# blubs/OpenGLRaytracer

Hardware: AMD Instinct MI355X
Metric: primary Mrays/s at 1920×1080; achieved HBM GB/s vs peak; 1/2/4/8-GPU scaling (higher is better)
Workload: dtype f32

## Files before the change

openglraytracer_amd/csrc/rt_api.cpp:

```cpp
#include <hip/hip_runtime.h>

#include <algorithm>
#include <climits>
#include <cmath>
#include <cstdio>
#include <cstring>
#include <new>
#include <string>
#include <vector>

#include "build_id.h"
#include "rt_internal.h"

namespace rtamd {

namespace {
thread_local std::string g_error;
}

void set_error(const std::string &msg) { g_error = msg; }

int hip_fail(const char *what, hipError_t e) {
    set_error(std::string(what) + ": " + hipGetErrorString(e));
    return RT_ERR_HIP;
// ... 203 lines not shown
            e = hipMemcpyAsync(static_cast<float4 *>(nb) + base, olist.data(), olist.size(), hipMemcpyHostToDevice,
                               ctx->stream);
        if (e == hipSuccess) e = hipStreamSynchronize(ctx->stream);
        if (e == hipSuccess) e = await_scene_uses(scene, ctx->stream);
        if (e != hipSuccess) {
            (void)hipFreeAsync(nb, ctx->stream);
            return hip_fail("origin lists upload", e);
        }
        (void)hipFreeAsync(scene->dev.blob, ctx->stream);
        drop_scene_uses(scene);
        scene->dev.blob = nb;
        scene->capacity_units = static_cast<int32_t>(units);
    } else {
        e = hipMemcpyAsync(static_cast<float4 *>(scene->dev.blob) + base, olist.data(), olist.size(),
                           hipMemcpyHostToDevice, ctx->stream);
        if (e == hipSuccess) e = hipStreamSynchronize(ctx->stream);
        if (e != hipSuccess) return hip_fail("origin lists upload", e);
    }
    scene->dev.off_olist = static_cast<int32_t>(base);
    return RT_OK;
}

}

extern "C" {

const char *rt_last_error(void) { return g_error.c_str(); }

int rt_debug_scene_blob(const rt_object *objs, int n_objs, const rt_material *mats, int n_mats,
                        const rt_light *lights, int n_lights, void *out, long long cap, int32_t *meta) {
    std::vector<float4> blob;
    DeviceScene ds;
    const int rc = build_scene(objs, n_objs, mats, n_mats, lights, n_lights, blob, ds, true);
    if (rc != RT_OK) return rc;
    const long long bytes = static_cast<long long>(blob.size() * sizeof(float4));
    if (out && cap >= bytes) std::memcpy(out, blob.data(), static_cast<size_t>(bytes));
    if (meta) {
        const int32_t m[24] = {ds.blob_units, ds.off_spheres, ds.off_smeta, ds.off_boxes, ds.off_mats,
                               ds.off_lights, ds.off_lightmat, ds.off_bvh, ds.n_bvh, ds.off_blink, ds.off_cone,
                               ds.off_dmask, ds.dmask_n, ds.dmask_bytes, ds.off_gmask, ds.gmask_words,
                               ds.off_glist, ds.n_spheres, ds.n_boxes, ds.n_mats, ds.n_lights, ds.off_olist,
                               0, 0};
        std::memcpy(meta, m, sizeof m);
    }
    return static_cast<int>(bytes);
}
int rt_debug_launch_shape_n(const int32_t *f, int n) {
    if (!f || (n != 15 && n != 23)) return RT_ERR_INVALID;
    LaunchParams p{};
    int resident = 0;
    if (n == 23) {
        static const FrameView views[1] = {};
        static const float4 consts[1] = {};
        static int32_t sched[1] = {};
        p.n_views = f[15];
        p.views_dev = f[16] ? views : nullptr;
        p.consts_dev = f[16] ? consts : nullptr;
        p.sched = f[18] ? sched : nullptr;
        p.persistent0 = f[17] ? 0 : f[19];
        resident = f[20];
        p.shape_cull = f[21];
        p.off_dmask = f[22] > 0 ? 0 : -1;
        p.dmask_bytes = f[22];
        p.dmask_n = kShapeMaskTexels;
    }
    p.shape_launch = f[1];
    p.width = f[2];
    p.height = f[3];
    p.row_begin = f[4];
    p.n_rows = f[5];
    p.block_rows = f[6];
    p.n_shards = f[7];
    p.shard = f[8];
    p.out_format = f[9];
    p.n_frame_consts = f[10];
    p.cam_short = f[11];
    p.slice_begin = f[12];
    p.slice_rows = f[13];
    p.spp = f[14];
    return launch_shape(p, f[0], resident);
}
int rt_debug_launch_shape(const int32_t *f) { return rt_debug_launch_shape_n(f, 15); }
int rt_debug_last_queued(const rt_context *ctx) { return ctx ? (ctx->last_queued ? 1 : 0) : RT_ERR_INVALID; }
const char *rt_version(void) { return "openglraytracer_amd 0.3 (gfx950, " RT_BUILD_ID ")"; }

int rt_create(int device, rt_context **out) {
    if (!out) { set_error("rt_create: null out"); return RT_ERR_INVALID; }
    *out = nullptr;
    int n = 0;
    hipError_t e = hipGetDeviceCount(&n);
    if (e != hipSuccess || n <= 0) {
        set_error("rt_create: no HIP device");
        return RT_ERR_NO_DEVICE;
    }
    if (device < 0 || device >= n) {
        set_error("rt_create: device " + std::to_string(device) + " out of range");
        return RT_ERR_NO_DEVICE;
    }
    if ((e = hipSetDevice(device)) != hipSuccess) return hip_fail("hipSetDevice", e);
    rt_context *ctx = new (std::nothrow) rt_context;
    if (!ctx) { set_error("rt_create: out of memory"); return RT_ERR_NOMEM; }
    ctx->device = device;
    for (hipEvent_t &ev : ctx->sched_done)
        if ((e = hipEventCreateWithFlags(&ev, hipEventDisableTiming)) != hipSuccess) {
            rt_destroy(ctx);
            return hip_fail("rt_create", e);
        }
    if ((e = hipStreamCreateWithFlags(&ctx->stream, hipStreamDefault)) != hipSuccess ||
        (e = hipEventCreate(&ctx->ev0)) != hipSuccess || (e = hipEventCreate(&ctx->ev1)) != hipSuccess ||
        (e = hipDeviceGetAttribute(&ctx->n_cu, hipDeviceAttributeMultiprocessorCount, device)) != hipSuccess ||
        (e = hipMalloc(&ctx->sched, sizeof(int32_t) * kSchedInts * kSchedSlots)) != hipSuccess ||
        (e = hipMemset(ctx->sched, 0, sizeof(int32_t) * kSchedInts * kSchedSlots)) != hipSuccess ||
        (e = allow_large_lds(kMaxLds)) != hipSuccess) {
        rt_destroy(ctx);
        return hip_fail("rt_create", e);
    }
    int rc = check_kernarg_block(ctx->stream);
    if (rc != RT_OK) {
        rt_destroy(ctx);
        return rc;
    }
    *out = ctx;
    return RT_OK;
}

void rt_destroy(rt_context *ctx) {
    if (!ctx) return;
    (void)hipSetDevice(ctx->device);
    if (ctx->stream) (void)hipStreamSynchronize(ctx->stream);
    for (rt_scene *s : ctx->scenes) s->ctx = nullptr;
    for (hipEvent_t ev : ctx->sched_done)
        if (ev) (void)hipEventDestroy(ev);
    if (ctx->staging) (void)hipFree(ctx->staging);
    for (int s = 0; s < kBatchSlots; ++s) {
        if (ctx->batch_dev[s]) (void)hipFree(ctx->batch_dev[s]);
        if (ctx->batch_host[s]) (void)hipHostFree(ctx->batch_host[s]);
        if (ctx->batch_done[s]) (void)hipEventDestroy(ctx->batch_done[s]);
    }
    if (ctx->sched) (void)hipFree(ctx->sched);
    if (ctx->ev0) (void)hipEventDestroy(ctx->ev0);
    if (ctx->ev1) (void)hipEventDestroy(ctx->ev1);
    if (ctx->stream) (void)hipStreamDestroy(ctx->stream);
    delete ctx;
}

int rt_scene_create(rt_context *ctx, const rt_object *objs, int n_objs, const rt_material *mats, int n_mats,
                    const rt_light *lights, int n_lights, rt_scene **out) {
    if (!out) { set_error("rt_scene_create: null out"); return RT_ERR_INVALID; }
    *out = nullptr;
    if (!ctx || (n_objs > 0 && !objs) || n_objs < 0 || n_objs > RT_MAX_OBJECTS || !mats || n_mats <= 0 ||
        n_mats > RT_MAX_MATERIALS || n_lights < 0 || n_lights > RT_MAX_LIGHTS || (n_lights > 0 && !lights)) {
        set_error("rt_scene_create: bad arguments");
        return RT_ERR_INVALID;
    }
    std::vector<float4> blob;
    DeviceScene ds;
    int rc = build_scene(objs, n_objs, mats, n_mats, lights, n_lights, blob, ds);
    if (rc != RT_OK) return rc;
    LaunchParams probe{};
    probe.blob_units = ds.blob_units;
    probe.n_spheres = ds.n_spheres;
    probe.n_boxes = ds.n_boxes;
    const size_t lds = lds_bytes(probe);
    if (lds > kMaxLds) {
        set_error("rt_scene_create: scene needs " + std::to_string(lds) + " B of LDS (> 160 KiB)");
        return RT_ERR_UNSUPPORTED;
// ... 493 lines not shown
```

openglraytracer_amd/csrc/rt_internal.h:

```cpp
#pragma once

#include <hip/hip_runtime.h>

#include <cstdint>
#include <memory>
#include <string>
#include <vector>

#include "../../include/rt.h"

namespace rtamd {

struct SphereRec {
    float cx, cy, cz, rr;
};
struct SphereMeta {
    int32_t obj_index;
    int32_t material;
    float radius;
    int32_t pad;
};

struct BoxRec {
    float w2l[12];
// ... 45 lines not shown
constexpr int kOListSlots = 25;
constexpr int kOListRecordBytes = 32;
#ifndef RT_OLIST_FROM
#define RT_OLIST_FROM 33
#endif
constexpr int kOListMinSpheres = RT_OLIST_FROM;
constexpr float kOListBoundUnit = 1.0f / 256.0f;
struct BvhNode {
    float lo[3];
    int32_t skip;
    float hi[3];
    int32_t leaf;
};
static_assert(sizeof(BvhNode) == 32, "BvhNode layout");
constexpr int kBvhOctants = 8;

struct LightRec {
    float pos[3];
    float dead;
};

struct FrameView {
    float unproj[16];
    float proj[16];
    float origin[3];
    int32_t cull;
    const void *blob;
};
constexpr int kMaxViews = 8;
constexpr int kBatchSlots = 4;
constexpr int kMaxFrameConsts = 272;
constexpr int kMaxViewConsts = 256;
constexpr size_t kMaxLds = 160 * 1024;

struct LaunchParams {
    FrameView view[kMaxViews];
    int32_t n_views;
    int32_t width, height;
    int32_t row_begin, n_rows;
    int32_t block_rows, n_shards, shard;
    int32_t n_spheres, n_boxes, n_mats, n_lights;
    const void *scene;
    float4 *out;
    int32_t off_spheres, off_smeta, off_boxes, off_mats, off_lights, off_lightmat;
    int32_t off_bvh, n_bvh;
    int32_t off_blink;
    int32_t off_cone;
    int32_t off_dmask, dmask_n;
    int32_t dmask_bytes;
    int32_t off_gmask, gmask_words;
    int32_t off_glist;
    int32_t blob_units;
    int32_t spp, sample0, jitter;
    uint32_t seed;
    int32_t *sched;
    int32_t n_cu;
    int32_t out_format;
    int32_t n_frame_consts;
    int32_t cam_short;
    int32_t slice_begin, slice_rows;
    const FrameView *views_dev;
    const float4 *consts_dev;
    float4 frame_consts[kMaxFrameConsts];
    int32_t off_olist;
    int32_t dmask_box;
    int32_t off_bplane;
    int32_t shape_cull;
    int32_t scene_room;
    int32_t lean_views;
    int32_t shape_launch;
    int32_t persistent0;
};
static_assert(sizeof(LaunchParams) == 5808, "kernel argument block: the hidden arguments' offsets");
static_assert(sizeof(LaunchParams) <= 6144, "kernel argument block");
constexpr int kShapeMaskBytes = 15;
constexpr int kShapeMaskTexels = 12;
constexpr int kShapeRoom = 16;
constexpr int kShapeWide = 32;
int scene_shape(const LaunchParams &p, int max_depth);
constexpr int kLaunchPlain = 1;
constexpr int kLaunchPersistent = 2;
int launch_shape(const LaunchParams &p, int max_depth, int resident = 0);
#ifndef RT_CHUNK0
#define RT_CHUNK0 8
#endif
constexpr int kChunk0 = RT_CHUNK0;
#ifndef RT_TAIL_TILES0
#define RT_TAIL_TILES0 4
#endif
constexpr int kTailTiles0 = RT_TAIL_TILES0;
constexpr int kPersistentMinTilesPerWave = 192;
int persistent_groups(const LaunchParams &p, int resident);
constexpr bool kLeanViews(int shape) { return (shape & kShapeWide) != 0; }
inline int view_units(const LaunchParams &p) { return (p.lean_views ? 1 : 2) * p.n_spheres + p.n_boxes; }
constexpr int kQueues = 32;
constexpr int kQueueStride = 64;
constexpr int kSchedInts = 2 * kQueues * kQueueStride;
constexpr int kSchedSlots = 64;

struct DeviceScene {
    void *blob = nullptr;
    int32_t blob_units = 0;
    int32_t off_spheres = 0, off_smeta = 0, off_boxes = 0, off_mats = 0, off_lights = 0, off_lightmat = 0;
    int32_t off_bvh = 0, n_bvh = 0, off_blink = 0, off_cone = 0;
    int32_t off_dmask = -1, dmask_n = 0, dmask_bytes = 4;
    int32_t dmask_box = 0;
    int32_t off_bplane = -1;
    int32_t off_gmask = -1, gmask_words = 0, off_glist = -1;
    int32_t off_olist = -1;
    int32_t olist_eligible = 0;
    int32_t n_spheres = 0, n_boxes = 0, n_mats = 0, n_lights = 0;
    int32_t room = 0;
};

void host_frame_setup(LaunchParams &p, const float4 *const *blobs);
int host_view_consts(const LaunchParams &p, const FrameView &V, const float4 *blob, float4 *out);
bool fill_view(const rt_context *ctx, const rt_view &view, int width, int height, FrameView &out);

float gl_sin(float a);
float gl_cos(float a);
void reference_orbit(float time, float *speed, float pos[3], float *yaw);
void reference_view_gl(float time, float unproj[16], float view[16]);
void reference_box_transforms(const float pos[3], const float ang[3], float l2w[16], float w2l[16], float nrm[9]);

hipError_t launch_render(LaunchParams &p, int max_depth, hipStream_t stream);
size_t lds_bytes(const LaunchParams &p);
int queued_views(const LaunchParams &p, int max_depth);
int check_kernarg_block(hipStream_t stream);

void set_error(const std::string &msg);
int hip_fail(const char *what, hipError_t e);
struct UseEvent {
    hipEvent_t ev = nullptr;
    UseEvent() = default;
    UseEvent(const UseEvent &) = delete;
    UseEvent &operator=(const UseEvent &) = delete;
    ~UseEvent() {
        if (ev) (void)hipEventDestroy(ev);
    }
};
int check_render_args(const rt_context *ctx, const rt_scene *scene, int width, int height, int max_depth);
LaunchParams base_params(const rt_context *ctx, const rt_scene *scene, const rt_view *views, int n_views,
                         int width, int height);
int launch(rt_context *ctx, LaunchParams &p, int max_depth, hipStream_t stream);
int ensure_origin_lists(rt_context *ctx, const rt_scene *scene, int max_depth);
int note_scene_use(const rt_scene *scene, hipStream_t stream, std::shared_ptr<UseEvent> *shared = nullptr);
inline size_t surface_bytes(int fmt) { return fmt == RT_OUTPUT_RGBA8 ? 4 : (fmt == RT_OUTPUT_RGB32F ? 12 : 16); }

}

struct rt_context {
    int device = 0;
    hipStream_t stream = nullptr;
    hipEvent_t ev0 = nullptr, ev1 = nullptr;
    float4 *staging = nullptr;
    size_t staging_px = 0;
    bool timed = false;
    int culling = 1;
    int timing = 1;
    int output = RT_OUTPUT_RGBA32F;
    int host_consts = 1;
    int origin_lists = 1;
    int scene_shapes = 1;
    int launch_shapes = 1;
    int persistent0 = 1;
    void *batch_dev[rtamd::kBatchSlots] = {};
    void *batch_host[rtamd::kBatchSlots] = {};
    hipEvent_t batch_done[rtamd::kBatchSlots] = {};
    bool batch_used[rtamd::kBatchSlots] = {};
    unsigned batch_next = 0;
    int n_cu = 0;
    int32_t *sched = nullptr;
    unsigned sched_next = 0;
    hipEvent_t sched_done[rtamd::kSchedSlots] = {};
    bool sched_used[rtamd::kSchedSlots] = {};
    bool last_queued = false;
    std::vector<struct rt_scene *> scenes;
};

struct rt_scene {
    int device = 0;
// ... 15 lines not shown
```

openglraytracer_amd/csrc/rt_kernel.hip:

```cpp
#include <hip/hip_runtime.h>

#include <algorithm>
#include <climits>
#include <cstdint>
#include <string>

#include "rt_internal.h"

namespace rtamd {
namespace {

constexpr int kWavesX = 2, kWavesY = 2;
constexpr int kTileX = 8 * kWavesX, kTileY = 8 * kWavesY;
constexpr int kThreads = 64 * kWavesX * kWavesY;

struct v3 {
    float x, y, z;
};
__device__ __forceinline__ v3 mk(float x, float y, float z) { return {x, y, z}; }
__device__ __forceinline__ v3 add(v3 a, v3 b) { return {a.x + b.x, a.y + b.y, a.z + b.z}; }
__device__ __forceinline__ v3 sub(v3 a, v3 b) { return {a.x - b.x, a.y - b.y, a.z - b.z}; }
__device__ __forceinline__ v3 muls(v3 a, float s) { return {a.x * s, a.y * s, a.z * s}; }
__device__ __forceinline__ v3 sel(bool c, v3 a, v3 b) { return {c ? a.x : b.x, c ? a.y : b.y, c ? a.z : b.z}; }
__device__ __forceinline__ float dot(v3 a, v3 b) { return a.x * b.x + (a.y * b.y + a.z * b.z); }
// ... 828 lines not shown
            const int s = base + __builtin_ctzll(mask);
            mask &= mask - 1;
            exact(s);
            if (!wave_any(need && !hit)) return hit;
        }
    }
    return hit;
}

__device__ __forceinline__ bool occluded(const Scene &S, v3 start, v3 dir, v3 p, v3 L, int light, int slot,
                                         uint64_t mask, bool need, const uint4 *pre = nullptr) {
    RT_CYC(kCycShadow);
    const bool hit = occluded_impl(S, start, dir, p, L, light, slot, mask, need, pre);
    RT_CYC_AFTER(kCycPhong, hit ? 1 : 0);
    return hit;
}

struct Collision {
    v3 p, n;
    bool inside;
    int material;
};

template <bool kPrimary>
__device__ __forceinline__ Collision resolve_impl(const Scene &S, const Ray &r, const Hit &h, bool valid) {
    Collision c;
    c.p = mk(0.0f, 0.0f, 0.0f);
    c.n = mk(0.0f, 0.0f, 1.0f);
    c.inside = false;
    c.material = 0;
    if (!valid) return c;
    if (h.slot >= 0) {
        const float4 sp = S.sph[h.slot];
        const v3 pos = mk(sp.x, sp.y, sp.z);
        c.material = S.smeta[h.slot].y;
        c.p = add(r.start, muls(r.dir, h.t));
        c.n = normalize(sub(c.p, pos));
        c.inside = h.info & 1;
        if (c.inside) c.n = muls(c.n, -1.0f);
    } else {
        const BoxRec &B = S.box[~h.slot];
        c.material = B.material;
        v3 rs;
        if (kPrimary) {
            const float4 bc = S.box_cam[~h.slot];
            rs = mk(bc.x, bc.y, bc.z);
        } else {
            rs = xform_point(B.w2l, r.start);
        }
        const v3 rd = box_dir(B, r.dir);
        c.inside = h.info & 1;
        const int face = h.info >> 1;
        v3 n = mk(face == 0 ? 1.0f : 0.0f, face == 1 ? 1.0f : 0.0f, face == 2 ? 1.0f : 0.0f);
        if (comp(rd, face) > 0.0f) n = muls(n, -1.0f);
        const float *N = B.nrm;
        c.n = mk(N[0] * n.x + N[1] * n.y + N[2] * n.z, N[3] * n.x + N[4] * n.y + N[5] * n.z,
                 N[6] * n.x + N[7] * n.y + N[8] * n.z);
        const v3 lp = add(rs, muls(rd, h.t));
        c.p = xform_point(B.l2w, lp);
    }
    return c;
}
template <bool kPrimary>
__device__ __forceinline__ Collision resolve(const Scene &S, const Ray &r, const Hit &h, bool valid) {
    RT_CYC(kCycResolve);
    const Collision c = resolve_impl<kPrimary>(S, r, h, valid);
    RT_CYC_AFTER(kCycWalk, c.p.x);
    return c;
}

#ifdef RT_PHASE_TRACE
constexpr unsigned kPhaseWaves = 1u << 17;
__device__ unsigned long long rt_phase_buf[kPhaseWaves * 16];
#define RT_PHASE(k)                                                                                        \
    do {                                                                                                    \
        const unsigned long long now_ = __builtin_amdgcn_s_memrealtime();                                   \
        const unsigned wg_ = (blockIdx.y * gridDim.x + blockIdx.x) * (kThreads / 64) + (threadIdx.x >> 6); \
        if ((threadIdx.x & 63) == 0 && wg_ < kPhaseWaves) rt_phase_buf[wg_ * 16 + (k)] = now_;              \
    } while (0)
#define RT_PHASE_AFTER(k, v)                     \
    do {                                         \
        if ((v) != -12345) RT_PHASE(k);      \
    } while (0)
#else
#define RT_PHASE_AFTER(k, v) \
    do {                     \
    } while (0)
#define RT_PHASE(k) \
    do {            \
    } while (0)
#endif

template <bool kUni = false>
__device__ __forceinline__ v3 phong_impl(const Scene &S, const Ray &r, const Collision &c, bool valid, int umat = 0) {
#if defined(RT_UNIFORM_MAT) && !defined(RT_UNIFORM_MAT_LM_ONLY)
    const MatRec m = kUni ? cload(S.cmat + umat) : S.mat[c.material];
#else
    const MatRec &m = S.mat[c.material];
#endif
    float4 dif = make_float4(0.0f, 0.0f, 0.0f, 0.0f), spe = dif;
    const v3 view = normalize_unit(muls(r.dir, -1.0f));
    int slot = -1;
    for (int j = 0; j < S.nl; ++j) {
        const LightRec L = cload(S.clight + j);
        if (L.dead != 0.0f) continue;
        ++slot;
        const v3 lpos = mk(L.pos[0], L.pos[1], L.pos[2]);
        const v3 sdir = sub(lpos, c.p);
        int ptexel = -1;
        uint4 pre = make_uint4(0u, 0u, 0u, 0u);
        if (S.glist) {
            ptexel = valid ? direction_texel(kGMaskTexels, muls(sdir, -1.0f)) : -1;
            if (ptexel >= 0) pre = S.glist[static_cast<size_t>(slot) * 6 * kGMaskTexels * kGMaskTexels + ptexel];
        }
        const v3 ldir = normalize(sdir);
        const float cos_theta = dot(ldir, c.n);
        const v3 nl = muls(ldir, -1.0f);
        const v3 lref = normalize_unit(sub(nl, muls(c.n, 2.0f * -cos_theta)));
        const float cos_phi = dot(view, lref);
#ifdef RT_UNIFORM_MAT
        const LightMatRec q = kUni ? cload(S.clm + (umat * S.nl + j)) : S.lm[c.material * S.nl + j];
#else
        const LightMatRec &q = S.lm[c.material * S.nl + j];
#endif
        const float kd = gmax(cos_theta, 0.0f);
        const float xs = gmax(cos_phi, 0.0f);
        const bool need_pow = !((xs == 0.0f) & (m.shininess > 0.0f));
        float ks = 0.0f;
        if (wave_any(need_pow && valid)) ks = need_pow ? glsl_pow_cos(xs, m.shininess) : 0.0f;
        const float4 nd = make_float4(dif.x + q.ld_md[0] * kd, dif.y + q.ld_md[1] * kd, dif.z + q.ld_md[2] * kd,
                                      dif.w + q.ld_md[3] * kd);
        const float4 ns = make_float4(spe.x + q.ls_ms[0] * ks, spe.y + q.ls_ms[1] * ks, spe.z + q.ls_ms[2] * ks,
                                      spe.w + q.ls_ms[3] * ks);
        const bool changes = (q.always != 0) | ((kd != 0.0f) & (q.d_nz != 0)) | ((ks != 0.0f) & (q.s_nz != 0));
        const bool need = valid && changes;
        if (j == 1) RT_PHASE(5);
#ifdef RT_ABLATE_SHADOW
        if (need) { dif = nd; spe = ns; }
        continue;
#endif
        if (wave_any(need)) {
            uint64_t smask = 0u;
            if (S.glist)
                smask = static_cast<uint64_t>(static_cast<int64_t>(ptexel));
            else if (S.gmask && need)
                smask = static_cast<uint64_t>(static_cast<int64_t>(direction_texel(kGMaskTexels, muls(sdir, -1.0f))));
            else if (S.dmask && !S.gmask)
                smask = direction_mask(S.dmask + slot * 6 * S.dmask_n * S.dmask_n * S.dmask_bytes, S.dmask_n,
                                       S.dmask_bytes, muls(sdir, -1.0f), S.ns + (S.dmask_box ? S.nb : 0));
            const bool shadowed = occluded(S, add(c.p, muls(c.n, 0.01f)), sdir, c.p, lpos, j, slot, smask, need,
                                           S.glist ? &pre : nullptr);
            if (need && !shadowed) {
                dif = nd;
                spe = ns;
            }
        }
    }
    RT_PHASE(6);
    const float px = ((m.amb_sum[0] + dif.x) + spe.x) + m.emissive[0];
    const float py = ((m.amb_sum[1] + dif.y) + spe.y) + m.emissive[1];
    const float pz = ((m.amb_sum[2] + dif.z) + spe.z) + m.emissive[2];
    const float pw = ((m.amb_sum[3] + dif.w) + spe.w) + m.emissive[3];
    return mk(px * pw, py * pw, pz * pw);
}
__device__ __forceinline__ v3 phong(const Scene &S, const Ray &r, const Collision &c, bool valid) {
    RT_CYC(kCycPhong);
    const v3 col = phong_impl(S, r, c, valid);
    RT_CYC_AFTER(kCycWalk, col.x);
    return col;
}

__device__ __forceinline__ v3 trace0(const Scene &S, const Ray &r, bool valid) {
// ... 353 lines not shown
        __builtin_assume(S.gmask != nullptr);
        __builtin_assume(S.glist != nullptr);
        __builtin_assume(S.olist != nullptr);
    }
    if constexpr ((kShape & kShapeRoom) != 0) {
        S.nb = 1;
        S.room = 1;
        S.dmask_box = 0;
        S.cbplane = nullptr;
    }
    RT_CYC(kCycRaygen);
    if (!wave_any(px.active)) return;
    const int x = px.x, y = px.y, local_row = px.local_row;
    const bool active = px.active;
    constexpr bool kPlain = (kLaunch & kLaunchPlain) != 0;
    static_assert(!kPlain || (kDepth == 0 && !kAccum && (kShape & kShapeMaskBytes) != 0),
                  "plain launches: the depth-0 shaped kernels, no accumulation");
    const int lr0 = (kPlain ? 0 : p.slice_begin) + wy * 8;
    S.tx0 = wx * 8;
    S.tx1 = S.tx0 + 7;
    if (kPlain || p.n_shards <= 0 || (p.block_rows % 8 == 0 && lr0 % 8 == 0)) {
        S.ty0 = output_row<kLaunch>(p, lr0);
        S.ty1 = S.ty0 + 7;
    } else {
        S.ty0 = INT_MAX;
        S.ty1 = INT_MIN;
        for (int i = 0; i < 8; ++i) {
            const int fy = output_row(p, lr0 + i);
            S.ty0 = fy < S.ty0 ? fy : S.ty0;
            S.ty1 = fy > S.ty1 ? fy : S.ty1;
        }
    }
    float4 *out = p.out + static_cast<size_t>(z) * p.n_rows * p.width;
    const uint32_t idx = static_cast<uint32_t>(local_row) * static_cast<uint32_t>(p.width) + static_cast<uint32_t>(x);

    if constexpr (!kAccum) {
        const Ray ray = have_pre ? pre : camera_ray<kLaunch>(p, V, x, y, 0.0f, 0.0f);
#if defined(RT_ABLATE_RAYGEN)
        (void)ray;
        const v3 col = mk(float(x), float(y), 0.0f);
#elif defined(RT_ABLATE_TRACE)
        const v3 col = ray.dir;
#else
        if constexpr (kDepth > 0) {
            trace_tree<kDepth>(S, ray, active, [&](v3 col) { store_pixel(p, z, idx, col); });
            return;
        }
        const v3 col = trace0(S, ray, active);
#endif
        RT_CYC_AFTER(kCycStore, col.x);
        if (active) store_pixel<kLaunch>(p, z, idx, col);
    } else {
        const uint32_t pixel = static_cast<uint32_t>(y) * static_cast<uint32_t>(p.width) + static_cast<uint32_t>(x);
        v3 acc = mk(0.0f, 0.0f, 0.0f);
        for (int smp = 0; smp < p.spp; ++smp) {
            const uint32_t sid = static_cast<uint32_t>(p.sample0 + smp);
            const float jx = p.jitter ? jitter_u(p.seed, sid, pixel, 0u) : 0.0f;
            const float jy = p.jitter ? jitter_u(p.seed, sid, pixel, 1u) : 0.0f;
            v3 col = mk(0.0f, 0.0f, 0.0f);
            if constexpr (kDepth == 0) col = trace0(S, camera_ray(p, V, x, y, jx, jy), active);
            else trace_tree<kDepth>(S, camera_ray(p, V, x, y, jx, jy), active, [&](v3 c) { col = c; });
            acc = add(acc, col);
        }
        if (active) {
            const float4 o = out[idx];
            out[idx] = make_float4(o.x + acc.x, o.y + acc.y, o.z + acc.z, o.w + 0.0f);
        }
    }
}

constexpr bool kQueuedDepth(int depth) { return depth >= 2; }

using LaunchArgs = const __attribute__((address_space(4))) LaunchParams *;
__device__ __forceinline__ const LaunchParams &launch_args() {
    LaunchArgs a = (LaunchArgs)__builtin_amdgcn_kernarg_segment_ptr();
    asm volatile("" : "+s"(a));
    return *(const LaunchParams *)a;
}
__device__ __forceinline__ float4 *persistent_slot(const LaunchParams &p, float4 *lds) {
    return lds + p.blob_units + __builtin_amdgcn_readfirstlane(threadIdx.x >> 6) * p.n_frame_consts;
}
__device__ __forceinline__ void persistent_refill(const LaunchParams &p, float4 *lds, int z) {
    float4 *const slot = persistent_slot(p, lds);
    __builtin_amdgcn_fence(__ATOMIC_RELEASE, "wavefront");
    __builtin_amdgcn_wave_barrier();
    int lane = threadIdx.x & 63;
    asm volatile("" : "+v"(lane));
    for (int i = lane; i < p.n_frame_consts; i += 64) slot[i] = p.consts_dev[z * p.n_frame_consts + i];
    __builtin_amdgcn_fence(__ATOMIC_ACQUIRE, "wavefront");
    __builtin_amdgcn_wave_barrier();
}
template <int kShape, int kLaunch>
__device__ __forceinline__ void persistent_tile(const LaunchParams &p, float4 *lds, int z, int wx, int wy) {
    const float4 *blob = static_cast<const float4 *>(p.scene);
    float4 *const slot = persistent_slot(p, lds);
    Scene S;
    S.sph = lds + p.off_spheres;
    S.smeta = reinterpret_cast<const int4 *>(lds + p.off_smeta);
    S.sph_cam = slot;
    S.sph_px = reinterpret_cast<const int4 *>(slot + p.n_spheres);
    S.box = reinterpret_cast<const BoxRec *>(lds + p.off_boxes);
    S.box_cam = slot + 2 * p.n_spheres;
    S.mat = reinterpret_cast<const MatRec *>(lds + p.off_mats);
    S.light = reinterpret_cast<const LightRec *>(lds + p.off_lights);
    S.lm = reinterpret_cast<const LightMatRec *>(lds + p.off_lightmat);
    S.bvh = lds + p.off_bvh;
    S.blink = reinterpret_cast<const uint32_t *>(lds + p.off_blink);
    S.cone = nullptr;
    S.dmask = reinterpret_cast<const char *>(lds + p.off_dmask);
    S.dmask_n = kShapeMaskTexels;
    S.dmask_bytes = kShape & kShapeMaskBytes;
    S.dmask_box = p.dmask_box;
    S.cbplane = p.off_bplane >= 0 ? (const __attribute__((address_space(4))) float4 *)(blob + p.off_bplane) : nullptr;
    S.gmask = nullptr;
    S.gwords = 0;
    S.glist = nullptr;
    S.olist = nullptr;
    S.cbox = (const __attribute__((address_space(4))) BoxRec *)(blob + p.off_boxes);
    S.clight = (const __attribute__((address_space(4))) LightRec *)(blob + p.off_lights);
#ifdef RT_UNIFORM_MAT
    S.cmat = (const __attribute__((address_space(4))) MatRec *)(blob + p.off_mats);
    S.clm = (const __attribute__((address_space(4))) LightMatRec *)(blob + p.off_lightmat);
#endif
    S.nbvh = 0;
    S.ns = p.n_spheres;
    S.nb = p.n_boxes;
    S.nl = p.n_lights;
    S.nm = p.n_mats;
    const FrameView V = cload((const __attribute__((address_space(4))) FrameView *)(p.views_dev) + z);
    const Ray none{mk(0.0f, 0.0f, 0.0f), mk(0.0f, 0.0f, 0.0f)};
    render_wave_tile<0, false, kShape, kLaunch>(p, S, V, wx, wy, z, wave_pixel<kLaunch>(p, wx, wy), none, false);
}
template <int kShape, int kLaunch>
__device__ __forceinline__ void render_persistent0(float4 *lds) {
    static_assert((kLaunch & kLaunchPlain) != 0 && (kShape & kShapeMaskBytes) != 0, "plain shaped launches");
    __builtin_amdgcn_s_setprio(1);
    {
        const LaunchParams &p = launch_args();
        const float4 *blob = static_cast<const float4 *>(p.scene);
        for (int i = threadIdx.x; i < p.blob_units; i += kThreads) lds[i] = blob[i];
    }
    __syncthreads();
    __builtin_amdgcn_s_setprio(0);
    const auto global_wave = [] {
        return static_cast<int>(blockIdx.x) * (kThreads / 64) + __builtin_amdgcn_readfirstlane(threadIdx.x >> 6);
    };
    const auto queue_waves = [](int q) {
        return (static_cast<int>(gridDim.x) * (kThreads / 64) - q + kQueues - 1) / kQueues;
    };
    int held = -1;
    int c = global_wave();
    for (;;) {
        int t, t_end, z, wx, wy;
        {
            const LaunchParams &p = launch_args();
            const int wtx = (p.width + 7) / 8, view_tiles = wtx * ((p.height + 7) / 8);
            const int total = view_tiles * p.n_views;
            const int tail_max = kTailTiles0 * static_cast<int>(gridDim.x) * (kThreads / 64);
            const int body = (total - (total < tail_max ? total : tail_max)) / kChunk0;
            if (c >= body + (total - body * kChunk0)) break;
            const int q = global_wave() % kQueues;
            int nxt = 0;
            if ((threadIdx.x & 63) == 0) nxt = atomicAdd(p.sched + q * kQueueStride, 1);
            t = c < body ? c * kChunk0 : body * kChunk0 + (c - body);
            t_end = c < body ? t + kChunk0 : t + 1;
            z = t / view_tiles;
            const int r = t - z * view_tiles;
            wy = r / wtx;
            wx = r - wy * wtx;
            if (z != held) persistent_refill(p, lds, z);
            held = z;
            c = (queue_waves(q) + __builtin_amdgcn_readfirstlane(nxt)) * kQueues + q;
        }
        for (; t < t_end; ++t) {
            const LaunchParams &p = launch_args();
            if (z != held) persistent_refill(p, lds, z);
            held = z;
            persistent_tile<kShape, kLaunch>(p, lds, z, wx, wy);
            if (++wx == (p.width + 7) / 8) {
                wx = 0;
                if (++wy == (p.height + 7) / 8) {
                    wy = 0;
                    ++z;
                }
            }
        }
    }
    const LaunchParams &p = launch_args();
    const int q = global_wave() % kQueues;
    if ((threadIdx.x & 63) == 0 && atomicAdd(p.sched + (kQueues + q) * kQueueStride, 1) == queue_waves(q) - 1) {
        atomicExch(p.sched + q * kQueueStride, 0);
        atomicExch(p.sched + (kQueues + q) * kQueueStride, 0);
    }
}

template <int kDepth, bool kAccum, bool kDev = false, int kShape = 0, int kLaunch = 0>
__global__ __launch_bounds__(kThreads) RT_OCCUPANCY void render_kernel(LaunchParams p) {
    constexpr bool kPlain = (kLaunch & kLaunchPlain) != 0;
    extern __shared__ __attribute__((aligned(16))) float4 lds[];
    if constexpr ((kLaunch & kLaunchPersistent) != 0) {
        static_assert(kPlain && kDev && kDepth == 0 && !kAccum, "persistent: plain depth-0 device-view batches");
        render_persistent0<kShape, kLaunch>(lds);
        return;
    }
    __builtin_amdgcn_s_setprio(1);
    const bool queued = kQueuedDepth(kDepth) && !kDev && p.sched != nullptr;
    const int z = queued ? 0 : static_cast<int>(blockIdx.z);
    const int n_staged = queued ? p.n_views : 1;
    FrameView Vdev;
    if constexpr (kDev) Vdev = cload((const __attribute__((address_space(4))) FrameView *)(p.views_dev) + z);
    const FrameView &V = kDev ? Vdev : p.view[z];
    const int wave = __builtin_amdgcn_readfirstlane(threadIdx.x >> 6), lane = threadIdx.x & 63;
    RT_PHASE(0);
#ifdef RT_PHASE_TRACE
    {
        const unsigned wg_ = (blockIdx.y * gridDim.x + blockIdx.x) * (kThreads / 64) + (threadIdx.x >> 6);
        const unsigned hw = __builtin_amdgcn_s_getreg((31 << 11) | 4), xcc = __builtin_amdgcn_s_getreg((31 << 11) | 20);
        if ((threadIdx.x & 63) == 0 && wg_ < kPhaseWaves) {
            rt_phase_buf[wg_ * 16 + 8] = hw;
            rt_phase_buf[wg_ * 16 + 9] = xcc;
        }
    }
#endif
    const float4 *blob = static_cast<const float4 *>(V.blob ? V.blob : p.scene);
    const int tid = threadIdx.x;
    float4 first = make_float4(0.0f, 0.0f, 0.0f, 0.0f), fc = first;
    if (tid < p.blob_units) first = blob[tid];
    static_assert(kMaxViewConsts <= kThreads, "one record per thread");
    constexpr bool kLean = kLeanViews(kShape);
    const int skip = kLean ? p.n_spheres : 0, keep = p.n_frame_consts - skip;
    if (tid < keep) fc = (kDev ? p.consts_dev : p.frame_consts)[z * p.n_frame_consts + skip + tid];
    float4 *const views = lds + p.blob_units;
    float4 *sph_cam = kLean ? nullptr : views;
    int4 *sph_px = reinterpret_cast<int4 *>(views + (kLean ? 0 : p.n_spheres));
    float4 *box_cam = reinterpret_cast<float4 *>(sph_px + p.n_spheres);
    const int own_wx = static_cast<int>(blockIdx.x) * kWavesX + wave % kWavesX;
    const int own_wy = static_cast<int>(blockIdx.y) * kWavesY + wave / kWavesX;
    const Pixel own = wave_pixel<kLaunch>(p, own_wx, own_wy);
    RT_PHASE_AFTER(14, own.y);
    Ray own_ray{mk(0.0f, 0.0f, 0.0f), mk(0.0f, 0.0f, 0.0f)};
    if (!queued && !kAccum) own_ray = camera_ray<kLaunch>(p, V, own.x, own.y, 0.0f, 0.0f);
    RT_PHASE_AFTER(15, own_ray.dir.x + own_ray.dir.y + own_ray.dir.z);
    RT_PHASE(10);
    if (tid < p.blob_units) lds[tid] = first;
    RT_PHASE(11);
    for (int i = tid + kThreads; i < p.blob_units; i += kThreads) lds[i] = blob[i];
    const int view_units = (kLean ? 1 : 2) * p.n_spheres + p.n_boxes;
    if (kPlain || p.n_frame_consts > 0) {
        if (tid < keep) views[tid] = fc;
        if (kLean) {
            for (int i = tid + keep; i < n_staged * keep; i += kThreads) {
                const int k = i / keep;
                views[i] = p.frame_consts[k * p.n_frame_consts + skip + (i - k * keep)];
            }
        } else {
            for (int i = tid + p.n_frame_consts; i < n_staged * p.n_frame_consts; i += kThreads)
                views[i] = p.frame_consts[i];
        }
    } else {
        frame_setup(p, V, sph_cam, sph_px, box_cam);
        for (int k = 1; k < n_staged; ++k) {
            float4 *c = views + k * view_units;
            int4 *px = reinterpret_cast<int4 *>(c + (kLean ? 0 : p.n_spheres));
            frame_setup(p, p.view[k], kLean ? nullptr : c, px, reinterpret_cast<float4 *>(px + p.n_spheres));
        }
    }
    RT_PHASE(12);
#ifdef RT_STATS
    if (lane < kStats) rt_stats_lds[wave][lane] = 0u;
#endif
#ifdef RT_CYCLES
    if (lane <= kCycPhases) rt_cyc_lds[wave][lane] = lane == kCycPhases ? __builtin_amdgcn_s_memtime() : 0u;
// ... 151 lines not shown
}

template <bool kAccum, bool kDev, int kShape>
hipError_t launch_shaped0(LaunchParams &p, hipStream_t stream) {
    if constexpr (!kAccum) {
        if ((launch_shape(p, 0) & kLaunchPlain) != 0) {
            if constexpr (kDev) {
                constexpr int kPersistent = kLaunchPlain | kLaunchPersistent;
                const size_t lds = persistent_lds_bytes(p);
                if (p.persistent0 > 0 && p.sched && lds <= kMaxLds && p.n_cu > 0) {
                    const void *fn = reinterpret_cast<const void *>(&render_kernel<0, false, true, kShape, kPersistent>);
                    const int groups = persistent_groups(p, groups_per_cu(fn, lds) * p.n_cu);
                    if (groups > 0) {
                        p.lean_views = 0;
                        hipLaunchKernelGGL((render_kernel<0, false, true, kShape, kPersistent>), dim3(groups),
                                           dim3(kThreads), lds, stream, p);
                        return hipGetLastError();
                    }
                }
            }
            return launch_kernel<0, false, kDev, kShape, kLaunchPlain>(p, stream);
        }
    }
    return launch_kernel<0, kAccum, kDev, kShape>(p, stream);
}
template <bool kAccum, bool kDev>
hipError_t launch_depth0(LaunchParams &p, hipStream_t stream) {
    switch (scene_shape(p, 0)) {
        case 2: return launch_shaped0<kAccum, kDev, 2>(p, stream);
        case 4: return launch_shaped0<kAccum, kDev, 4>(p, stream);
        case 8: return launch_shaped0<kAccum, kDev, 8>(p, stream);
        case 2 | kShapeRoom: return launch_shaped0<kAccum, kDev, 2 | kShapeRoom>(p, stream);
        case 4 | kShapeRoom: return launch_shaped0<kAccum, kDev, 4 | kShapeRoom>(p, stream);
        case 8 | kShapeRoom: return launch_shaped0<kAccum, kDev, 8 | kShapeRoom>(p, stream);
        default: return launch_kernel<0, kAccum, kDev, 0>(p, stream);
    }
}

template <int kDepth>
hipError_t launch_deep(LaunchParams &p, hipStream_t stream) {
    switch (scene_shape(p, kDepth)) {
        case kShapeWide: return launch_kernel<kDepth, false, false, kShapeWide>(p, stream);
        case kShapeWide | kShapeRoom: return launch_kernel<kDepth, false, false, kShapeWide | kShapeRoom>(p, stream);
        default: return launch_kernel<kDepth, false, false, 0>(p, stream);
    }
}

template <int kDepth>
hipError_t launch_depth(LaunchParams &p, hipStream_t stream) {
    if (p.views_dev) {
        if constexpr (kDepth == 0) {
            if (p.spp == 0) return launch_depth0<false, true>(p, stream);
        } else if constexpr (kDepth == 1) {
            if (p.spp == 0) return launch_kernel<kDepth, false, true>(p, stream);
        }
        return hipErrorInvalidValue;
    }
    if constexpr (kDepth == 0) return p.spp > 0 ? launch_depth0<true, false>(p, stream) : launch_depth0<false, false>(p, stream);
    if constexpr (kDepth >= 2) {
        if (p.spp == 0) return launch_deep<kDepth>(p, stream);
    }
    return p.spp > 0 ? launch_kernel<kDepth, true>(p, stream) : launch_kernel<kDepth, false>(p, stream);
}

}

int scene_shape(const LaunchParams &p, int max_depth) {
    if (!p.shape_cull) return 0;
    const int box = p.n_boxes == 1 && p.scene_room ? kShapeRoom : 0;
    if (max_depth == 0) {
        if (p.off_dmask < 0 || (p.dmask_bytes != 2 && p.dmask_bytes != 4 && p.dmask_bytes != 8) ||
            p.dmask_n != kShapeMaskTexels)
            return 0;
        return p.dmask_bytes | box;
    }
    if (max_depth >= 2) {
        if (p.off_gmask < 0 || p.off_glist < 0 || p.off_olist < 0) return 0;
        return kShapeWide | box;
    }
    return 0;
}

int persistent_groups(const LaunchParams &p, int resident) {
#if defined(RT_STATS) || defined(RT_CYCLES) || defined(RT_PHASE_TRACE)
    return 0;
#endif
    if (p.persistent0 <= 0 || (launch_shape(p, 0) & kLaunchPlain) == 0 || scene_shape(p, 0) == 0) return 0;
    if (!p.views_dev || !p.consts_dev || p.n_views <= kMaxViews || !p.sched) return 0;
    const bool forced = p.persistent0 >= 8;
    const int groups = forced && p.persistent0 < resident ? p.persistent0 : resident;
    const long long waves = static_cast<long long>(groups) * (kThreads / 64);
    const long long tiles = static_cast<long long>((p.width + 7) / 8) * ((p.height + 7) / 8) * p.n_views;
    if (waves < kQueues || tiles >= (1ll << 30)) return 0;
    if (!forced && tiles < kPersistentMinTilesPerWave * waves) return 0;
    return groups;
}

int launch_shape(const LaunchParams &p, int max_depth, int resident) {
    if (resident > 0) {
        const int shape = launch_shape(p, max_depth);
        return shape | (shape != 0 && persistent_groups(p, resident) > 0 ? kLaunchPersistent : 0);
    }
    if (!p.shape_launch || max_depth != 0 || p.spp > 0) return 0;
    const int slice_rows = p.slice_rows > 0 ? p.slice_rows : p.n_rows;
    const int slice_begin = p.slice_rows > 0 ? p.slice_begin : 0;
    const bool plain = p.n_shards <= 0 && p.row_begin == 0 && p.n_rows == p.height && slice_begin == 0 &&
                       slice_rows == p.n_rows && p.out_format == RT_OUTPUT_RGBA32F && p.cam_short == 1 &&
                       p.n_frame_consts > 0 && p.width >= 2 && p.height >= 2;
    return plain ? kLaunchPlain : 0;
}

size_t lds_bytes(const LaunchParams &p) {
    return (static_cast<size_t>(p.blob_units) + view_units(p)) * sizeof(float4);
}

int queued_views(const LaunchParams &p, int max_depth) {
    const void *fn = nullptr;
    switch (max_depth) {
        case 2: fn = reinterpret_cast<const void *>(&render_kernel<2, false>); break;
        case 3: fn = reinterpret_cast<const void *>(&render_kernel<3, false>); break;
        case 4: fn = reinterpret_cast<const void *>(&render_kernel<4, false>); break;
        case 5: fn = reinterpret_cast<const void *>(&render_kernel<5, false>); break;
        case 6: fn = reinterpret_cast<const void *>(&render_kernel<6, false>); break;
        case 7: fn = reinterpret_cast<const void *>(&render_kernel<7, false>); break;
        case 8: fn = reinterpret_cast<const void *>(&render_kernel<8, false>); break;
        case 9: fn = reinterpret_cast<const void *>(&render_kernel<9, false>); break;
        default: return 1;
    }
    static_assert(!kQueuedDepth(1) && kQueuedDepth(2), "queued from depth 2");
    return queued_views_for(fn, p);
}

hipError_t launch_render(LaunchParams &p, int max_depth, hipStream_t stream) {
    if (p.slice_rows <= 0) {
        p.slice_begin = 0;
        p.slice_rows = p.n_rows;
    }
    switch (max_depth) {
        case 0: return launch_depth<0>(p, stream);
        case 1: return launch_depth<1>(p, stream);
        case 2: return launch_depth<2>(p, stream);
        case 3: return launch_depth<3>(p, stream);
        case 4: return launch_depth<4>(p, stream);
        case 5: return launch_depth<5>(p, stream);
        case 6: return launch_depth<6>(p, stream);
        case 7: return launch_depth<7>(p, stream);
        case 8: return launch_depth<8>(p, stream);
        case 9: return launch_depth<9>(p, stream);
        default: return hipErrorInvalidValue;
    }
}

__global__ void kernarg_probe(LaunchParams p, float4 *out) {
    if (threadIdx.x == 0 && blockIdx.x == 0) {
        out[0] = p.frame_consts[kMaxFrameConsts - 1];
        out[1] = make_float4(__int_as_float(p.n_frame_consts), __int_as_float(p.out_format), 0.0f, 0.0f);
    }
}

int check_kernarg_block(hipStream_t stream) {
    LaunchParams p{};
    p.frame_consts[kMaxFrameConsts - 1] = make_float4(1.5f, -2.25f, 3.125f, 4096.0f);
    p.n_frame_consts = 0x5a5a;
    p.out_format = 0x3c3c;
    float4 *d = nullptr, h[2] = {};
    hipError_t e = hipMalloc(&d, sizeof h);
    if (e == hipSuccess) {
// ... 93 lines not shown
```

Baseline: 82740.

## Use geometric chunk schedule and rotated queue mapping in persistent depth-0 kernel

Replaces the fixed-size bulk chunk plus single-tile tail with a schedule that halves the chunk size from 16 down to single tiles as the remaining work shrinks. Waves are now mapped to queue counters through a rotation so neighbouring groups spread across different counters. The atomic fetch of the next chunk is moved to after the current chunk's tiles finish instead of before. The goal is less contention on the atomics and better load balance at the tail. It also adds phase-trace instrumentation and debug entry points.

```diff
diff --git a/openglraytracer_amd/csrc/rt_api.cpp b/openglraytracer_amd/csrc/rt_api.cpp
--- a/openglraytracer_amd/csrc/rt_api.cpp
+++ b/openglraytracer_amd/csrc/rt_api.cpp
@@ -309,6 +309,20 @@
 }
 int rt_debug_launch_shape(const int32_t *f) { return rt_debug_launch_shape_n(f, 15); }
 int rt_debug_last_queued(const rt_context *ctx) { return ctx ? (ctx->last_queued ? 1 : 0) : RT_ERR_INVALID; }
+int rt_debug_persistent_chunk(int c, int total, int waves, int32_t *out) {
+    if (!out || c < 0 || total < 0 || total >= (1 << 30) || waves <= 0) return RT_ERR_INVALID;
+    const ChunkRange r = persistent_chunk(c, total, waves);
+    out[0] = r.t;
+    out[1] = r.t_end;
+    return RT_OK;
+}
+int rt_debug_persistent_queue(int g, int waves, int32_t *out) {
+    if (!out || g < 0 || waves <= 0 || g >= waves) return RT_ERR_INVALID;
+    out[0] = persistent_queue(g);
+    out[1] = persistent_queue_waves(out[0], waves);
+    out[2] = persistent_first_chunk(g);
+    return RT_OK;
+}
 const char *rt_version(void) { return "openglraytracer_amd 0.3 (gfx950, " RT_BUILD_ID ")"; }
 
 int rt_create(int device, rt_context **out) {
diff --git a/openglraytracer_amd/csrc/rt_internal.h b/openglraytracer_amd/csrc/rt_internal.h
--- a/openglraytracer_amd/csrc/rt_internal.h
+++ b/openglraytracer_amd/csrc/rt_internal.h
@@ -151,13 +151,25 @@
 constexpr int kLaunchPersistent = 2;
 int launch_shape(const LaunchParams &p, int max_depth, int resident = 0);
 #ifndef RT_CHUNK0
-#define RT_CHUNK0 8
+#define RT_CHUNK0 16
 #endif
 constexpr int kChunk0 = RT_CHUNK0;
-#ifndef RT_TAIL_TILES0
-#define RT_TAIL_TILES0 4
-#endif
-constexpr int kTailTiles0 = RT_TAIL_TILES0;
+static_assert(kChunk0 >= 2 && kChunk0 <= 32 && (kChunk0 & (kChunk0 - 1)) == 0, "bulk chunk: a power of two, 2..32");
+struct ChunkRange {
+    int t, t_end;
+};
+__host__ __device__ inline ChunkRange persistent_chunk(int c, int total, int waves) {
+    int start = 0;
+#pragma unroll
+    for (int s = kChunk0; s >= 2; s >>= 1) {
+        const int left = (total - start) / s - waves;
+        const int n = left > 0 ? left : 0;
+        if (c < n) return {start + c * s, start + c * s + s};
+        c -= n;
+        start += n * s;
+    }
+    return c < total - start ? ChunkRange{start + c, start + c + 1} : ChunkRange{total, total};
+}
 constexpr int kPersistentMinTilesPerWave = 192;
 int persistent_groups(const LaunchParams &p, int resident);
 constexpr bool kLeanViews(int shape) { return (shape & kShapeWide) != 0; }
@@ -166,6 +178,17 @@
 constexpr int kQueueStride = 64;
 constexpr int kSchedInts = 2 * kQueues * kQueueStride;
 constexpr int kSchedSlots = 64;
+#ifndef RT_QUEUE_ROTATE0
+#define RT_QUEUE_ROTATE0 5
+#endif
+constexpr int kQueueRotate0 = RT_QUEUE_ROTATE0;
+static_assert((kQueues & (kQueues - 1)) == 0, "the queue arithmetic masks with kQueues - 1");
+__host__ __device__ inline int persistent_queue(int g) { return (g + kQueueRotate0 * (g / kQueues)) & (kQueues - 1); }
+__host__ __device__ inline int persistent_queue_waves(int q, int waves) {
+    const int rounds = waves / kQueues, rest = waves & (kQueues - 1);
+    return rounds + (((q - kQueueRotate0 * rounds) & (kQueues - 1)) < rest ? 1 : 0);
+}
+__host__ __device__ inline int persistent_first_chunk(int g) { return (g & ~(kQueues - 1)) + persistent_queue(g); }
 
 struct DeviceScene {
     void *blob = nullptr;
diff --git a/openglraytracer_amd/csrc/rt_kernel.hip b/openglraytracer_amd/csrc/rt_kernel.hip
--- a/openglraytracer_amd/csrc/rt_kernel.hip
+++ b/openglraytracer_amd/csrc/rt_kernel.hip
@@ -934,12 +934,46 @@
     do {                                         \
         if ((v) != -12345) RT_PHASE(k);      \
     } while (0)
+#define RT_PHASE_WAVE (blockIdx.x * (kThreads / 64) + (threadIdx.x >> 6))
+#define RT_PHASE_LANE0 ((threadIdx.x & 63) == 0 && RT_PHASE_WAVE < kPhaseWaves)
+#define RT_PHASE_SLOT(k) rt_phase_buf[RT_PHASE_WAVE * 16 + (k)]
+#define RT_PHASE_ONCE(k)                                                                 \
+    do {                                                                                 \
+        const unsigned long long now_ = __builtin_amdgcn_s_memrealtime();                \
+        if (RT_PHASE_LANE0 && RT_PHASE_SLOT(k) == 0) RT_PHASE_SLOT(k) = now_;   \
+    } while (0)
+#define RT_PHASE_COUNT(k, v)                                   \
+    do {                                                       \
+        if (RT_PHASE_LANE0) RT_PHASE_SLOT(k) += (v);  \
+    } while (0)
+#define RT_PHASE_CLOCK(name) const unsigned long long name = __builtin_amdgcn_s_memrealtime()
+#define RT_PHASE_SPAN(k, k2, t0_)                                                     \
+    do {                                                                              \
+        const unsigned long long d_ = __builtin_amdgcn_s_memrealtime() - (t0_);      \
+        if (RT_PHASE_LANE0) {                                                \
+            RT_PHASE_SLOT(k) += 1;                                                    \
+            RT_PHASE_SLOT((k) + 1) += d_;                                             \
+            if (d_ > RT_PHASE_SLOT(k2)) RT_PHASE_SLOT(k2) = d_;                       \
+        }                                                                             \
+    } while (0)
 #else
 #define RT_PHASE_AFTER(k, v) \
     do {                     \
     } while (0)
 #define RT_PHASE(k) \
     do {            \
+    } while (0)
+#define RT_PHASE_ONCE(k) \
+    do {                 \
+    } while (0)
+#define RT_PHASE_COUNT(k, v) \
+    do {                     \
+    } while (0)
+#define RT_PHASE_CLOCK(name) \
+    do {                     \
+    } while (0)
+#define RT_PHASE_SPAN(k, k2, t0_) \
+    do {                          \
     } while (0)
 #endif
 
@@ -1459,6 +1493,7 @@
 }
 __device__ __forceinline__ void persistent_refill(const LaunchParams &p, float4 *lds, int z) {
     float4 *const slot = persistent_slot(p, lds);
+    RT_PHASE_CLOCK(refill_t0);
     __builtin_amdgcn_fence(__ATOMIC_RELEASE, "wavefront");
     __builtin_amdgcn_wave_barrier();
     int lane = threadIdx.x & 63;
@@ -1466,6 +1501,7 @@
     for (int i = lane; i < p.n_frame_consts; i += 64) slot[i] = p.consts_dev[z * p.n_frame_consts + i];
     __builtin_amdgcn_fence(__ATOMIC_ACQUIRE, "wavefront");
     __builtin_amdgcn_wave_barrier();
+    RT_PHASE_SPAN(10, 12, refill_t0);
 }
 template <int kShape, int kLaunch>
 __device__ __forceinline__ void persistent_tile(const LaunchParams &p, float4 *lds, int z, int wx, int wy) {
@@ -1512,6 +1548,12 @@
 __device__ __forceinline__ void render_persistent0(float4 *lds) {
     static_assert((kLaunch & kLaunchPlain) != 0 && (kShape & kShapeMaskBytes) != 0, "plain shaped launches");
     __builtin_amdgcn_s_setprio(1);
+    RT_PHASE(0);
+#ifdef RT_PHASE_TRACE
+    if (RT_PHASE_LANE0) {
+        RT_PHASE_SLOT(8) = __builtin_amdgcn_s_getreg((31 << 11) | 4) | (unsigned long long)__builtin_amdgcn_s_getreg((31 << 11) | 20) << 32;
+    }
+#endif
     {
         const LaunchParams &p = launch_args();
         const float4 *blob = static_cast<const float4 *>(p.scene);
@@ -1519,40 +1561,40 @@
     }
     __syncthreads();
     __builtin_amdgcn_s_setprio(0);
+    RT_PHASE(13);
     const auto global_wave = [] {
         return static_cast<int>(blockIdx.x) * (kThreads / 64) + __builtin_amdgcn_readfirstlane(threadIdx.x >> 6);
     };
     const auto queue_waves = [](int q) {
-        return (static_cast<int>(gridDim.x) * (kThreads / 64) - q + kQueues - 1) / kQueues;
+        return persistent_queue_waves(q, static_cast<int>(gridDim.x) * (kThreads / 64));
     };
     int held = -1;
-    int c = global_wave();
+    int c = persistent_first_chunk(global_wave());
     for (;;) {
         int t, t_end, z, wx, wy;
         {
             const LaunchParams &p = launch_args();
             const int wtx = (p.width + 7) / 8, view_tiles = wtx * ((p.height + 7) / 8);
             const int total = view_tiles * p.n_views;
-            const int tail_max = kTailTiles0 * static_cast<int>(gridDim.x) * (kThreads / 64);
-            const int body = (total - (total < tail_max ? total : tail_max)) / kChunk0;
-            if (c >= body + (total - body * kChunk0)) break;
-            const int q = global_wave() % kQueues;
-            int nxt = 0;
-            if ((threadIdx.x & 63) == 0) nxt = atomicAdd(p.sched + q * kQueueStride, 1);
-            t = c < body ? c * kChunk0 : body * kChunk0 + (c - body);
-            t_end = c < body ? t + kChunk0 : t + 1;
+            const ChunkRange r_c = persistent_chunk(c, total, static_cast<int>(gridDim.x) * (kThreads / 64));
+            if (r_c.t >= r_c.t_end) break;
+            t = r_c.t;
+            t_end = r_c.t_end;
             z = t / view_tiles;
             const int r = t - z * view_tiles;
             wy = r / wtx;
             wx = r - wy * wtx;
+            RT_PHASE_ONCE(1);
+            if (t_end - t == 1) RT_PHASE_ONCE(14);
+            RT_PHASE_COUNT(15, 1);
             if (z != held) persistent_refill(p, lds, z);
             held = z;
-            c = (queue_waves(q) + __builtin_amdgcn_readfirstlane(nxt)) * kQueues + q;
         }
         for (; t < t_end; ++t) {
             const LaunchParams &p = launch_args();
             if (z != held) persistent_refill(p, lds, z);
             held = z;
+            RT_PHASE_COUNT(9, 1);
             persistent_tile<kShape, kLaunch>(p, lds, z, wx, wy);
             if (++wx == (p.width + 7) / 8) {
                 wx = 0;
@@ -1562,9 +1604,17 @@
                 }
             }
         }
-    }
+        {
+            const LaunchParams &p = launch_args();
+            const int q = persistent_queue(global_wave());
+            int nxt = 0;
+            if ((threadIdx.x & 63) == 0) nxt = atomicAdd(p.sched + q * kQueueStride, 1);
+            c = (queue_waves(q) + __builtin_amdgcn_readfirstlane(nxt)) * kQueues + q;
+        }
+    }
+    RT_PHASE(7);
     const LaunchParams &p = launch_args();
-    const int q = global_wave() % kQueues;
+    const int q = persistent_queue(global_wave());
     if ((threadIdx.x & 63) == 0 && atomicAdd(p.sched + (kQueues + q) * kQueueStride, 1) == queue_waves(q) - 1) {
         atomicExch(p.sched + q * kQueueStride, 0);
         atomicExch(p.sched + (kQueues + q) * kQueueStride, 0);
@@ -1882,7 +1932,7 @@
 }
 
 int persistent_groups(const LaunchParams &p, int resident) {
-#if defined(RT_STATS) || defined(RT_CYCLES) || defined(RT_PHASE_TRACE)
+#if defined(RT_STATS) || defined(RT_CYCLES)
     return 0;
 #endif
     if (p.persistent0 <= 0 || (launch_shape(p, 0) & kLaunchPlain) == 0 || scene_shape(p, 0) == 0) return 0;
```

Result: faster. 84790 (median of 6 runs) (+2.5%).
